# microsoft/GenerativeImage2Text

Hardware: AMD Instinct MI355X
Metric: captions/sec whole-node (GIT_BASE 224px bs=64/GPU greedy len=20) (higher is better)
Workload: dtype f16; 1 GPU; GIT_BASE 224px bs=64/GPU greedy max_len=20 frames=1; global_batch=64, parallelism=dp1, decode_steps_per_caption=19, seq_len_returned=20, hip_graph=True, contexts_in_flight=4, layernorm_folded=True, library=libgitmi_f16.so, encoder_chains=2, schedule=mixed

## Files before the change

### generativeimage2text_amd/csrc/kernels_attn.hip

```cpp
#include "gitmi_common.h"
#include "launchers.h"
#include <type_traits>

namespace gitmi {

constexpr int HD = 64;

template <typename T>
__global__ __launch_bounds__(256) void attn_full_valu_kernel(AttnFullArgs a) {
    __shared__ float Ks[64][HD + 1];
    __shared__ float Vs[64][HD + 1];
    __shared__ float qs[16][HD];
    __shared__ float ps[16][64];

    const int tid = threadIdx.x, lane = tid & 63, wave = tid >> 6;
    const int h = blockIdx.y, b = blockIdx.z;
    const int q0 = blockIdx.x * 16;
    const T* Q = reinterpret_cast<const T*>(a.q);
    const T* K = reinterpret_cast<const T*>(a.k);
    const T* V = reinterpret_cast<const T*>(a.v);
    T* O = reinterpret_cast<T*>(a.out);
    const size_t base_row = (size_t)b * a.N;
    const int n = a.ntok ? a.ntok[b] : a.N;
    if (q0 >= n) {
// ... 49 lines not shown
            for (int key = 0; key < 64; ++key) o += ps[qi][key] * Vs[key][lane];
            o_acc[j] = o;
        }
    }
#pragma unroll
    for (int j = 0; j < 4; ++j) {
        const int qr = q0 + wave * 4 + j;
        if (qr < a.N) st<T>(O + (base_row + qr) * a.ldo + h * HD + lane, qr < n ? o_acc[j] / l_run[j] : 0.f);
    }
}

constexpr int FA_LDK = HD + 8;
constexpr int FA_LDV = 64 + 8;

__global__ __launch_bounds__(256) void attn_full_mfma_kernel(AttnFullArgs a) {
    __shared__ __attribute__((aligned(16))) bf16_t Ks[64 * FA_LDK];
    __shared__ __attribute__((aligned(16))) bf16_t Vt[HD * FA_LDV];

    constexpr int QT = 4;
    const int tid = threadIdx.x, lane = tid & 63, wave = tid >> 6;
    const int l15 = lane & 15, lg = lane >> 4;
    const int h = blockIdx.y, b = blockIdx.z;
    const int qbase = blockIdx.x * 256;
    const bf16_t* Q = reinterpret_cast<const bf16_t*>(a.q);
    const bf16_t* K = reinterpret_cast<const bf16_t*>(a.k);
    const bf16_t* V = reinterpret_cast<const bf16_t*>(a.v);
    bf16_t* O = reinterpret_cast<bf16_t*>(a.out);
    const size_t base_row = (size_t)b * a.N;
    const int n = a.ntok ? a.ntok[b] : a.N;

    bf16x8_t qf[QT][2];
    f32x4_t o_acc[QT][4];
    float m_run[QT], l_run[QT];
#pragma unroll
    for (int t = 0; t < QT; ++t) {
        int qr = qbase + (t * 4 + wave) * 16 + l15;
        qr = qr < n ? qr : n - 1;
        const bf16_t* qp = Q + (base_row + qr) * a.ldq + h * HD + lg * 8;
        qf[t][0] = *reinterpret_cast<const bf16x8_t*>(qp);
        qf[t][1] = *reinterpret_cast<const bf16x8_t*>(qp + 32);
#pragma unroll
        for (int dt = 0; dt < 4; ++dt) o_acc[t][dt] = f32x4_t{0.f, 0.f, 0.f, 0.f};
        m_run[t] = -INFINITY;
        l_run[t] = 0.f;
    }

    const int ld_row = tid >> 3;
    const int ld_c = (tid & 7) * 8;

    const int kend = qbase < n ? n : 0;
    for (int kt = 0; kt < kend; kt += 64) {
        __syncthreads();
#pragma unroll
        for (int it = 0; it < 2; ++it) {
            const int key = ld_row + it * 32;
            int kr = kt + key;
            kr = kr < n ? kr : n - 1;
            const u32x4_t kc = *reinterpret_cast<const u32x4_t*>(K + (base_row + kr) * a.ldk + h * HD + ld_c);
            const u32x4_t vc = *reinterpret_cast<const u32x4_t*>(V + (base_row + kr) * a.ldv + h * HD + ld_c);
            *reinterpret_cast<u32x4_t*>(Ks + key * FA_LDK + ld_c) = kc;
#pragma unroll
            for (int e = 0; e < 4; ++e) {
                Vt[(ld_c + 2 * e) * FA_LDV + key] = (bf16_t)(vc[e] & 0xffffu);
                Vt[(ld_c + 2 * e + 1) * FA_LDV + key] = (bf16_t)(vc[e] >> 16);
            }
        }
        __syncthreads();

#pragma unroll
        for (int t = 0; t < QT; ++t) {
            if (qbase + (t * 4 + wave) * 16 >= n) continue;
            f32x4_t s_acc[4];
#pragma unroll
            for (int st_ = 0; st_ < 4; ++st_) {
                s_acc[st_] = f32x4_t{0.f, 0.f, 0.f, 0.f};
#pragma unroll
                for (int ks = 0; ks < 2; ++ks) {
                    const bf16x8_t kf = *reinterpret_cast<const bf16x8_t*>(Ks + (st_ * 16 + l15) * FA_LDK + ks * 32 + lg * 8);
                    s_acc[st_] = mfma16(kf, qf[t][ks], s_acc[st_]);
                }
            }
            float tmax = -INFINITY;
#pragma unroll
            for (int st_ = 0; st_ < 4; ++st_)
#pragma unroll
                for (int r = 0; r < 4; ++r) {
                    const int key = kt + st_ * 16 + lg * 4 + r;
                    const float sv = key < n ? s_acc[st_][r] * a.scale : -INFINITY;
                    s_acc[st_][r] = sv;
                    tmax = fmaxf(tmax, sv);
                }
            tmax = fmaxf(tmax, __shfl_xor(tmax, 16, 64));
            tmax = fmaxf(tmax, __shfl_xor(tmax, 32, 64));
            const float m_new = fmaxf(m_run[t], tmax);
            const float alpha = fast_exp(m_run[t] - m_new);
            float psum = 0.f;
#pragma unroll
            for (int st_ = 0; st_ < 4; ++st_)
#pragma unroll
                for (int r = 0; r < 4; ++r) {
                    const float p = fast_exp(s_acc[st_][r] - m_new);
                    s_acc[st_][r] = p;
                    psum += p;
                }
            psum += __shfl_xor(psum, 16, 64);
            psum += __shfl_xor(psum, 32, 64);
            l_run[t] = l_run[t] * alpha + psum;
            m_run[t] = m_new;
#pragma unroll
            for (int dt = 0; dt < 4; ++dt)
#pragma unroll
                for (int r = 0; r < 4; ++r) o_acc[t][dt][r] *= alpha;

#pragma unroll
            for (int hf = 0; hf < 2; ++hf) {
                bf16x8_t pf;
                {
                    union { bf16x8_t v; uint32_t u[4]; } pk;
                    pk.u[0] = pack2bf(s_acc[2 * hf][0], s_acc[2 * hf][1]);
                    pk.u[1] = pack2bf(s_acc[2 * hf][2], s_acc[2 * hf][3]);
                    pk.u[2] = pack2bf(s_acc[2 * hf + 1][0], s_acc[2 * hf + 1][1]);
                    pk.u[3] = pack2bf(s_acc[2 * hf + 1][2], s_acc[2 * hf + 1][3]);
                    pf = pk.v;
                }
#pragma unroll
                for (int dt = 0; dt < 4; ++dt) {
                    union { bf16x8_t v; uint2 h2[2]; } vf;
                    const bf16_t* vp = Vt + (dt * 16 + l15) * FA_LDV + hf * 32 + lg * 4;
                    vf.h2[0] = *reinterpret_cast<const uint2*>(vp);
                    vf.h2[1] = *reinterpret_cast<const uint2*>(vp + 16);
                    o_acc[t][dt] = mfma16(vf.v, pf, o_acc[t][dt]);
                }
            }
        }
    }

#pragma unroll
    for (int t = 0; t < QT; ++t) {
        const int qr = qbase + (t * 4 + wave) * 16 + l15;
        if (qr < a.N) {
            const float inv = qr < n ? 1.0f / l_run[t] : 0.f;
            bf16_t* op = O + (base_row + qr) * a.ldo + h * HD;
#pragma unroll
            for (int dt = 0; dt < 4; ++dt) {
                uint2 tt;
                tt.x = pack2bf(o_acc[t][dt][0] * inv, o_acc[t][dt][1] * inv);
                tt.y = pack2bf(o_acc[t][dt][2] * inv, o_acc[t][dt][3] * inv);
                *reinterpret_cast<uint2*>(op + dt * 16 + lg * 4) = tt;
            }
        }
    }
}

template <int NSUB, bool RAGGED = false>
__global__ __launch_bounds__(256, 2) void attn_full_mfma_short_kernel(AttnFullArgs a) {
    constexpr int NK = NSUB * 16;
    constexpr int NB = (NSUB + 1) / 2;
    constexpr int LDV = NB * 32 + 8;
    static_assert((LDV / 8) % 2 == 1, "V^T row stride must be an odd multiple of 16 bytes");
    __shared__ __attribute__((aligned(16))) bf16_t Ks[NK * FA_LDK];
    __shared__ __attribute__((aligned(16))) bf16_t Vt[HD * LDV];

    const int tid = threadIdx.x, lane = tid & 63, wave = tid >> 6;
    const int l15 = lane & 15, lg = lane >> 4;
    const int h = blockIdx.x, b = blockIdx.y;
    const bf16_t* Q = reinterpret_cast<const bf16_t*>(a.q);
    const bf16_t* K = reinterpret_cast<const bf16_t*>(a.k);
    const bf16_t* V = reinterpret_cast<const bf16_t*>(a.v);
    bf16_t* O = reinterpret_cast<bf16_t*>(a.out);
    const size_t base_row = (size_t)b * a.N;
    const int n = RAGGED ? a.ntok[b] : a.N;
    if constexpr (RAGGED) {
        for (int i = tid; i < (a.N - n) * 8; i += 256) {
            const int qr = n + (i >> 3);
            *reinterpret_cast<u32x4_t*>(O + (base_row + qr) * a.ldo + h * HD + (i & 7) * 8) = u32x4_t{0u, 0u, 0u, 0u};
        }
    }

#pragma unroll
    for (int it = 0; it < (NK * 8 + 255) / 256; ++it) {
        int idx = tid + it * 256;
        const bool ok = idx < NK * 8;
        idx = ok ? idx : NK * 8 - 1;
        const int key = idx >> 3, c = idx & 7;
        const int kr = key < n ? key : n - 1;
        const u32x4_t kc = *reinterpret_cast<const u32x4_t*>(K + (base_row + kr) * a.ldk + h * HD + c * 8);
        if (ok) *reinterpret_cast<u32x4_t*>(Ks + key * FA_LDK + c * 8) = kc;
    }
#pragma unroll
    for (int it = 0; it < (NB * 8 * 8 + 255) / 256; ++it) {
        int task = tid + it * 256;
        const bool ok = task < NB * 8 * 8;
        task = ok ? task : NB * 8 * 8 - 1;
        const int kg = task % (NB * 8), c = task / (NB * 8);
        u32x4_t vc[4];
#pragma unroll
        for (int e = 0; e < 4; ++e) {
            const int key = kg * 4 + e;
            const int kr = key < n ? key : n - 1;
            vc[e] = *reinterpret_cast<const u32x4_t*>(V + (base_row + kr) * a.ldv + h * HD + c * 8);
            if (key >= n) vc[e] = u32x4_t{0u, 0u, 0u, 0u};
        }
        if (ok) {
#pragma unroll
            for (int w = 0; w < 4; ++w) {
                uint2 even, odd;
                even.x = (vc[0][w] & 0xffffu) | (vc[1][w] << 16);
                even.y = (vc[2][w] & 0xffffu) | (vc[3][w] << 16);
                odd.x = (vc[0][w] >> 16) | (vc[1][w] & 0xffff0000u);
                odd.y = (vc[2][w] >> 16) | (vc[3][w] & 0xffff0000u);
                *reinterpret_cast<uint2*>(Vt + (c * 8 + 2 * w) * LDV + kg * 4) = even;
                *reinterpret_cast<uint2*>(Vt + (c * 8 + 2 * w + 1) * LDV + kg * 4) = odd;
            }
        }
    }
    __syncthreads();

    const int nqt = (n + 15) >> 4;
    const float c2 = a.scale * 1.4426950408889634f;

    auto process = [&](auto nt_c, int t0) {
        constexpr int NT = decltype(nt_c)::value;
        bf16x8_t qf[NT][2];
#pragma unroll
        for (int u = 0; u < NT; ++u) {
            int qr = (t0 + 4 * u) * 16 + l15;
            qr = qr < n ? qr : n - 1;
            const bf16_t* qp = Q + (base_row + qr) * a.ldq + h * HD + lg * 8;
            qf[u][0] = *reinterpret_cast<const bf16x8_t*>(qp);
            qf[u][1] = *reinterpret_cast<const bf16x8_t*>(qp + 32);
        }
        f32x4_t sacc[NT][NSUB];
#pragma unroll
        for (int st_ = 0; st_ < NSUB; ++st_) {
            const bf16x8_t kf0 = *reinterpret_cast<const bf16x8_t*>(Ks + (st_ * 16 + l15) * FA_LDK + lg * 8);
            const bf16x8_t kf1 = *reinterpret_cast<const bf16x8_t*>(Ks + (st_ * 16 + l15) * FA_LDK + 32 + lg * 8);
#pragma unroll
            for (int u = 0; u < NT; ++u) {
                sacc[u][st_] = mfma16(kf0, qf[u][0], f32x4_t{0.f, 0.f, 0.f, 0.f});
                sacc[u][st_] = mfma16(kf1, qf[u][1], sacc[u][st_]);
            }
            if constexpr (NSUB > 13) { if (st_ % 4 == 3) __builtin_amdgcn_sched_barrier(0); }
        }
        float inv_l[NT];
#pragma unroll
        for (int u = 0; u < NT; ++u) {
            if constexpr (RAGGED) {
#pragma unroll
                for (int st_ = 0; st_ < NSUB; ++st_)
#pragma unroll
                    for (int r = 0; r < 4; ++r)
                        if (st_ * 16 + lg * 4 + r >= n) sacc[u][st_][r] = -INFINITY;
            } else {
#pragma unroll
                for (int r = 0; r < 4; ++r)
                    if ((NSUB - 1) * 16 + lg * 4 + r >= a.N) sacc[u][NSUB - 1][r] = -INFINITY;
            }
            float m = -INFINITY;
#pragma unroll
            for (int st_ = 0; st_ < NSUB; ++st_)
#pragma unroll
                for (int r = 0; r < 4; ++r) m = fmaxf(m, sacc[u][st_][r]);
            m = fmaxf(m, __shfl_xor(m, 16, 64));
            m = fmaxf(m, __shfl_xor(m, 32, 64));
            const float mc = m * c2;
            float psum = 0.f;
#pragma unroll
            for (int st_ = 0; st_ < NSUB; ++st_)
#pragma unroll
                for (int r = 0; r < 4; ++r) {
                    const float p = __builtin_amdgcn_exp2f(sacc[u][st_][r] * c2 - mc);
                    sacc[u][st_][r] = p;
                    psum += p;
                }
            psum += __shfl_xor(psum, 16, 64);
            psum += __shfl_xor(psum, 32, 64);
            inv_l[u] = 1.0f / psum;
        }
        uint32_t pk2[NT][NSUB][2];
#pragma unroll
        for (int u = 0; u < NT; ++u)
#pragma unroll
            for (int st_ = 0; st_ < NSUB; ++st_) {
                pk2[u][st_][0] = pack2bf(sacc[u][st_][0], sacc[u][st_][1]);
                pk2[u][st_][1] = pack2bf(sacc[u][st_][2], sacc[u][st_][3]);
            }
        f32x4_t o_acc[NT][4];
#pragma unroll
        for (int u = 0; u < NT; ++u)
#pragma unroll
            for (int dt = 0; dt < 4; ++dt) o_acc[u][dt] = f32x4_t{0.f, 0.f, 0.f, 0.f};
#pragma unroll
        for (int blk = 0; blk < NB; ++blk) {
            bf16x8_t pf[NT];
#pragma unroll
            for (int u = 0; u < NT; ++u) {
                union { bf16x8_t v; uint32_t w[4]; } pk;
                pk.w[0] = pk2[u][2 * blk][0];
                pk.w[1] = pk2[u][2 * blk][1];
                const bool has1 = 2 * blk + 1 < NSUB;
                const int s1 = has1 ? 2 * blk + 1 : 0;
                pk.w[2] = has1 ? pk2[u][s1][0] : 0u;
                pk.w[3] = has1 ? pk2[u][s1][1] : 0u;
                pf[u] = pk.v;
            }
#pragma unroll
            for (int dt = 0; dt < 4; ++dt) {
                union { bf16x8_t v; uint2 h2[2]; } vf;
                const bf16_t* vp = Vt + (dt * 16 + l15) * LDV + blk * 32 + lg * 4;
                vf.h2[0] = *reinterpret_cast<const uint2*>(vp);
                vf.h2[1] = *reinterpret_cast<const uint2*>(vp + 16);
#pragma unroll
                for (int u = 0; u < NT; ++u)
                    o_acc[u][dt] = mfma16(vf.v, pf[u], o_acc[u][dt]);
            }
        }
#pragma unroll
        for (int u = 0; u < NT; ++u) {
            const int qr = (t0 + 4 * u) * 16 + l15;
            if (qr < n) {
                bf16_t* op = O + (base_row + qr) * a.ldo + h * HD;
#pragma unroll
                for (int dt = 0; dt < 4; ++dt) {
                    uint2 tt;
                    tt.x = pack2bf(o_acc[u][dt][0] * inv_l[u], o_acc[u][dt][1] * inv_l[u]);
                    tt.y = pack2bf(o_acc[u][dt][2] * inv_l[u], o_acc[u][dt][3] * inv_l[u]);
                    *reinterpret_cast<uint2*>(op + dt * 16 + lg * 4) = tt;
                }
            }
        }
    };

    for (int t0 = wave; t0 < nqt; t0 += 8) {
        if (t0 + 4 < nqt) process(std::integral_constant<int, 2>{}, t0);
        else process(std::integral_constant<int, 1>{}, t0);
    }
}

template <typename T>
__global__ void kv_repack_kernel(const T* __restrict__ qkv, T* __restrict__ kh, T* __restrict__ vh, int B, int N, int H,
                                 int d) {
    constexpr int CH = 16 / (int)sizeof(T);
    constexpr int CPH = HD / CH;
    const size_t per = (size_t)B * H * N * CPH;
    for (size_t i = blockIdx.x * (size_t)blockDim.x + threadIdx.x; i < 2 * per; i += (size_t)gridDim.x * blockDim.x) {
        const int kv = i >= per;
        size_t r = kv ? i - per : i;
        const int c = (int)(r % CPH); r /= CPH;
        const int n = (int)(r % N); r /= N;
        const int h = (int)(r % H);
        const int b = (int)(r / H);
        const T* src = qkv + ((size_t)b * N + n) * 3 * d + (kv ? 2 : 1) * d + h * HD + c * CH;
        T* dst = (kv ? vh : kh) + (((size_t)b * H + h) * N + n) * HD + c * CH;
        *reinterpret_cast<u32x4_t*>(dst) = *reinterpret_cast<const u32x4_t*>(src);
    }
}

template <typename T> struct Raw8;
template <> struct Raw8<bf16_t> {
    u32x4_t r;
    __device__ __forceinline__ void load(const bf16_t* p) { r = *reinterpret_cast<const u32x4_t*>(p); }
    __device__ __forceinline__ void load_nt(const bf16_t* p) { r = __builtin_nontemporal_load(reinterpret_cast<const u32x4_t*>(p)); }
    __device__ __forceinline__ void store(bf16_t* p) const { *reinterpret_cast<u32x4_t*>(p) = r; }
    __device__ __forceinline__ void zero() { r = u32x4_t{0u, 0u, 0u, 0u}; }
    __device__ __forceinline__ void get(float (&v)[8]) const {
#pragma unroll
        for (int i = 0; i < 4; ++i) {
            unpack2op(r[i], v[2 * i], v[2 * i + 1]);
        }
    }
};
template <> struct Raw8<float> {
    f32x4_t a, b;
    __device__ __forceinline__ void load(const float* p) {
        a = *reinterpret_cast<const f32x4_t*>(p);
        b = *reinterpret_cast<const f32x4_t*>(p + 4);
    }
    __device__ __forceinline__ void load_nt(const float* p) {
        a = __builtin_nontemporal_load(reinterpret_cast<const f32x4_t*>(p));
        b = __builtin_nontemporal_load(reinterpret_cast<const f32x4_t*>(p + 4));
    }
    __device__ __forceinline__ void store(float* p) const {
        *reinterpret_cast<f32x4_t*>(p) = a;
        *reinterpret_cast<f32x4_t*>(p + 4) = b;
    }
    __device__ __forceinline__ void zero() { a = f32x4_t{0.f, 0.f, 0.f, 0.f}; b = a; }
    __device__ __forceinline__ void get(float (&v)[8]) const {
#pragma unroll
        for (int i = 0; i < 4; ++i) { v[i] = a[i]; v[4 + i] = b[i]; }
    }
};

template <typename T, int KB, int PF = 8, int TI = 5>
__global__ __launch_bounds__(256) void attn_decode_kernel(AttnDecodeArgs a) {
    __shared__ float part[4][KB][HD + 2];

    const int tid = threadIdx.x;
    const int h = blockIdx.x, b = blockIdx.y, H = gridDim.x;
    const int k = a.beams;
    const T* QKV = reinterpret_cast<const T*>(a.qkv);
    const T* IMGK = reinterpret_cast<const T*>(a.img_k);
    const T* IMGV = reinterpret_cast<const T*>(a.img_v);
    T* TK = reinterpret_cast<T*>(a.txt_k);
    T* TV = reinterpret_cast<T*>(a.txt_v);
    T* O = reinterpret_cast<T*>(a.out);
    const int ld3 = 3 * a.d;
    const int row0 = b * k;
    const int grp = tid >> 3, sub = tid & 7;
    const int wave = tid >> 6;

    const int bi = a.img_of ? a.img_of[b] : b;
    const int n_img = a.ntok ? a.ntok[bi] : a.N_img;
    const T* kbase = IMGK + ((size_t)bi * H + h) * a.N_img * HD + sub * 8;
    const T* vbase = IMGV + ((size_t)bi * H + h) * a.N_img * HD + sub * 8;
    const int nt = a.pos + 1;

    int t_j[TI], t_s[TI], t_row[TI];
#pragma unroll
    for (int u = 0; u < TI; ++u) {
        const int it = grp + 32 * u;
        t_j[u] = it < k * nt ? it / nt : -1;
        t_s[u] = it < k * nt ? it % nt : 0;
        if constexpr (KB == 1) t_row[u] = row0;
        else t_row[u] = (t_j[u] >= 0 && t_s[u] != a.pos) ? a.kv_src[(size_t)(row0 + t_j[u]) * a.ld_src + t_s[u]] : 0;
    }
    Raw8<T> qr[KB];
#pragma unroll
    for (int j = 0; j < KB; ++j) {
        if (j < k) qr[j].load(QKV + (size_t)(row0 + j) * ld3 + h * HD + sub * 8);
        else qr[j].zero();
    }
    Raw8<T> kr[PF], vr[PF];
#pragma unroll
    for (int u = 0; u < PF; ++u) {
        const int n = grp + 32 * u;
        if (n < n_img && !(a.dbg & 1)) { kr[u].load_nt(kbase + (size_t)n * HD); vr[u].load_nt(vbase + (size_t)n * HD); }
        else { kr[u].zero(); vr[u].zero(); }
    }
    Raw8<T> tk[TI], tv[TI];
#pragma unroll
    for (int u = 0; u < TI; ++u) {
        if (t_j[u] < 0) { tk[u].zero(); tv[u].zero(); }
        else if (t_s[u] == a.pos) {
            const T* src = QKV + (size_t)(row0 + t_j[u]) * ld3 + a.d + h * HD + sub * 8;
            tk[u].load(src);
            tv[u].load(src + a.d);
        } else {
            const size_t off = ((size_t)t_row[u] * a.T_max + t_s[u]) * a.d + h * HD + sub * 8;
            tk[u].load(TK + off);
            tv[u].load(TV + off);
        }
    }
    if (tid < k * 8) {
        const int j = tid >> 3;
        const T* src = QKV + (size_t)(row0 + j) * ld3 + a.d + h * HD + sub * 8;
        const size_t dst = ((size_t)(row0 + j) * a.T_max + a.pos) * a.d + h * HD + sub * 8;
        Raw8<T> ck, cv;
        ck.load(src);
        cv.load(src + a.d);
        ck.store(TK + dst);
        cv.store(TV + dst);
    }

    float q[KB][8], m[KB], l[KB], o[KB][8];
// ... 191 lines not shown
```

### generativeimage2text_amd/engine.py

```python
from __future__ import annotations

import ctypes as C
import os
from typing import Dict, List, Mapping, Optional, Sequence, Tuple

import torch

_HERE = os.path.dirname(os.path.abspath(__file__))
LIB_PATH = os.path.join(_HERE, "libgitmi.so")
LIB_PATH_F16 = os.path.join(_HERE, "libgitmi_f16.so")
LIB_PATH_EXP = os.path.join(_HERE, "libgitmi_exp.so")
LIB_PATH_F16_EXP = os.path.join(_HERE, "libgitmi_f16_exp.so")

PREC_BF16, PREC_F32 = 0, 1
DTYPE_F32, DTYPE_BF16, DTYPE_F16 = 0, 1, 2
DTYPE_F16_STREAM = 3
SEARCH_AUTOREGRESSIVE, SEARCH_GENERATOR, SEARCH_TRIE = 0, 1, 2
SEARCH_SCORE = 3
SEARCH_ATTEND = 4
SEARCH_CONTEXT = 5
SEARCH_TREE_SCORE = 6
ACT_NONE, ACT_QUICKGELU, ACT_GELU_ERF = 0, 1, 2

EXPORTED_SYMBOLS = [
# ... 909 lines not shown
def from_frag(xf: torch.Tensor, rows: int) -> torch.Tensor:
    Rp, K = xf.shape
    return xf.reshape(Rp // 16, K // 32, 4, 16, 8).permute(0, 3, 1, 2, 4).reshape(Rp, K)[:rows].contiguous()


def _pad_vec(v: Optional[torch.Tensor], n: int) -> Optional[torch.Tensor]:
    if v is None:
        return None
    out = torch.zeros(n, dtype=v.dtype, device=v.device)
    out[:v.numel()] = v
    return out


def op_dgemm(A: torch.Tensor, W: torch.Tensor, bias: torch.Tensor, colsum: Optional[torch.Tensor] = None,
             stats: Optional[torch.Tensor] = None, eps: float = 1e-12, act: int = ACT_NONE,
             frag_out: bool = False, packed: bool = False, strips_per_wg: int = 0) -> torch.Tensor:
    lib = _op_library(A.dtype, W.dtype)
    if packed:
        Af, Wf, M, N, K = A, W, int(A.shape[0]), int(bias.numel()), int(A.shape[1])
        if stats is not None:
            M = int(stats.shape[1])
    else:
        M, K = A.shape
        N = W.shape[0]
        Af, Wf = to_frag(A, 64), to_frag(W)
    out = torch.empty((M + 15) // 16 * 16 if frag_out else M, N, device=A.device, dtype=A.dtype)
    strips = 0 if stats is None else int(stats.shape[0])
    _ck(lib.gitmi_op_dgemm(Af.data_ptr(), Wf.data_ptr(), bias.data_ptr(), _ptr(colsum), _ptr(stats), strips, eps,
                           out.data_ptr(), 1 if frag_out else 0, M, N, K, act, int(strips_per_wg), _stream()), lib)
    return from_frag(out, M) if (frag_out and not packed) else out


def op_dgemm_res(A: torch.Tensor, W: torch.Tensor, bias: torch.Tensor, res_x: torch.Tensor,
                 res_stats: Optional[torch.Tensor] = None, res_gamma: Optional[torch.Tensor] = None,
                 res_beta: Optional[torch.Tensor] = None, res_eps: float = 1e-12, packed: bool = False):
    lib = _op_library(A.dtype, W.dtype)
    M, N = res_x.shape
    K = A.shape[1]
    Af, Wf = (A, W) if packed else (to_frag(A, 64), to_frag(W))
    x = torch.empty(M, N, device=A.device, dtype=torch.float32)
    xb = torch.empty((M + 15) // 16 * 16, (N + 31) // 32 * 32, device=A.device, dtype=A.dtype)
    st = torch.empty(N // 16, M, 2, device=A.device, dtype=torch.float32)
    strips = 0 if res_stats is None else int(res_stats.shape[0])
    _ck(lib.gitmi_op_dgemm_res(Af.data_ptr(), Wf.data_ptr(), bias.data_ptr(), res_x.data_ptr(), _ptr(res_stats), strips,
                               _ptr(res_gamma), _ptr(res_beta), res_eps, x.data_ptr(), xb.data_ptr(), st.data_ptr(),
                               M, N, K, _stream()), lib)
    return x, (xb if packed else from_frag(xb, M)[:, :N].contiguous()), st


def op_dgemm_form(A: torch.Tensor, W: torch.Tensor, bias: torch.Tensor, M: Optional[int] = None, *, colsum=None, stats=None,
                  eps: float = 1e-12, act: int = ACT_NONE, frag_out: bool = False, out: Optional[torch.Tensor] = None,
                  res_x=None, res_stats=None, res_gamma=None, res_beta=None, res_eps: float = 1e-12, x=None, xb=None,
                  stats_out=None, packed: bool = False, rows_per_wg: int = 0, strips_per_wg: int = 0, no_row_walk: int = 0):
    lib = _exp_library(A.dtype, W.dtype)
    own = A.dtype
    if own == torch.float32:
        raise GitmiError(f"operands must be bf16 or fp16, got {A.dtype} / {W.dtype}")
    if packed:
        if M is None:
            raise ValueError("packed operands: M is required")
        Af, Wf = A, W
    else:
        M = int(A.shape[0]) if M is None else int(M)
        Af, Wf = to_frag(A, 64), to_frag(W)
    M, N, K = int(M), int(bias.numel()), int(A.shape[1])
    Mp = (M + 15) // 16 * 16
    producer = res_x is not None
    if producer:
        x = torch.empty(M, N, device=A.device, dtype=torch.float32) if x is None else x
        xb = torch.empty(Mp, (N + 31) // 32 * 32, device=A.device, dtype=own) if xb is None else xb
        stats_out = torch.empty(N // 16, M, 2, device=A.device, dtype=torch.float32) if stats_out is None else stats_out
    elif out is None:
        out = torch.empty(Mp if frag_out else M, N, device=A.device, dtype=own)
    _ck(_experiment_only(lib, "gitmi_debug_dgemm_form")(
        Af.data_ptr(), int(Af.shape[0]), Wf.data_ptr(), _ptr(bias), _ptr(colsum), _ptr(stats),
        0 if stats is None else int(stats.shape[0]), eps, _ptr(out), int(bool(frag_out)), int(act), _ptr(res_x), _ptr(res_stats),
        0 if res_stats is None else int(res_stats.shape[0]), _ptr(res_gamma), _ptr(res_beta), res_eps, _ptr(x), _ptr(xb),
        _ptr(stats_out), M, N, K, int(rows_per_wg), int(strips_per_wg), int(no_row_walk), _stream()), lib)
    return (x, xb, stats_out) if producer else out


def _vocab_head_call(A, W, bias, mtop, cols_per_wg, colsum, stats, want_logits, packed, rows, V, measurement=False):
    lib = _exp_library(A.dtype, W.dtype) if measurement else _op_library(A.dtype, W.dtype)
    K = A.shape[1]
    V = int(bias.numel()) if V is None else int(V)
    if packed:
        Af, Wf, M, bp, cp = A, W, int(rows), bias, colsum
    else:
        M = A.shape[0]
        Vp = (V + cols_per_wg - 1) // cols_per_wg * cols_per_wg
        Af, Wf, bp, cp = to_frag(A, 64), to_frag(W, cols_per_wg), _pad_vec(bias, Vp), _pad_vec(colsum, Vp)
    nparts = (V + cols_per_wg - 1) // cols_per_wg
    slots = 1 if mtop <= 1 else 2 if mtop <= 2 else 4 if mtop <= 4 else 8 if mtop <= 8 else 16
    pv = torch.empty(M, nparts, slots, device=A.device, dtype=torch.float32)
    pi = torch.empty(M, nparts, slots, device=A.device, dtype=torch.int32)
    pl = torch.empty(M, nparts, 2, device=A.device, dtype=torch.float32)
    lg = torch.empty(M, V, device=A.device, dtype=torch.float32) if want_logits else None
    strips = 0 if stats is None else int(stats.shape[0])
    keep = (Af, Wf, bp, cp)
    return lib, M, (Af.data_ptr(), Wf.data_ptr(), bp.data_ptr(), _ptr(cp), _ptr(stats), strips), (M, V, K, cols_per_wg, mtop), \
        (pv.data_ptr(), pi.data_ptr(), pl.data_ptr(), _ptr(lg)), (pv, pi, pl, lg), keep


def op_vocab_topm(A: torch.Tensor, W: torch.Tensor, bias: torch.Tensor, mtop: int, cols_per_wg: int = 128,
                  colsum: Optional[torch.Tensor] = None, stats: Optional[torch.Tensor] = None, eps: float = 1e-12,
                  suppress_tok: Optional[torch.Tensor] = None, want_logits: bool = False, packed: bool = False,
                  rows: Optional[int] = None, V: Optional[int] = None, max_wgs: int = 0):
    lib, _, ops, shape, outs, result, keep = _vocab_head_call(A, W, bias, mtop, cols_per_wg, colsum, stats, want_logits, packed, rows, V)
    _ck(lib.gitmi_op_vocab_topm(*ops, eps, *shape, _ptr(suppress_tok), *outs, int(max_wgs), _stream()), lib)
    return result


def op_vocab_topm_rules(A: torch.Tensor, W: torch.Tensor, bias: torch.Tensor, mtop: int, ids: Optional[torch.Tensor],
                        cur_len: int, plen: Optional[torch.Tensor], beams: int = 1, suppress_kind: int = 0,
                        rep_penalty: float = 0.0, cols_per_wg: int = 128, colsum: Optional[torch.Tensor] = None,
                        stats: Optional[torch.Tensor] = None, eps: float = 1e-12, want_logits: bool = False, packed: bool = False,
                        rows: Optional[int] = None, V: Optional[int] = None, max_wgs: int = 0):
    lib, M, ops, shape, outs, result, keep = _vocab_head_call(A, W, bias, mtop, cols_per_wg, colsum, stats, want_logits, packed, rows, V,
                                                              measurement=True)
    if ids is not None:
        ids = ids.to(device=A.device, dtype=torch.int32).contiguous()
        plen = plen.to(device=A.device, dtype=torch.int32).contiguous()
        if ids.dim() != 2 or ids.shape[0] != M or plen.numel() * beams != M:
            raise ValueError(f"ids {tuple(ids.shape)} / plen {tuple(plen.shape)} do not describe {M} rows of {beams} beams")
    _ck(_experiment_only(lib, "gitmi_debug_vocab_topm_rules")(
        *ops, eps, *shape, _ptr(ids), 0 if ids is None else int(ids.shape[1]), int(cur_len), _ptr(plen), int(beams),
        int(suppress_kind), float(rep_penalty), *outs, int(max_wgs), _stream()), lib)
    return result


def set_gemm_impl(impl: int) -> None:
    global _gemm_impl
    lib = load_library()
    _ck(_experiment_only(lib, "gitmi_debug_set_gemm_impl")(int(impl)), lib)
    _gemm_impl = int(impl)
    other = _libs.get("f16_exp")
    if other is not None and other is not lib:
        _ck(other.gitmi_debug_set_gemm_impl(int(impl)), other)


def op_attn_decode(qkv, img_k, img_v, txt_k, txt_v, kv_src, B, H, N_img, T_max, pos, beams, dbg=0):
    lib = _op_library(qkv.dtype, img_k.dtype, img_v.dtype, txt_k.dtype, txt_v.dtype, fp32_ok=True)
    R, d = B * beams, H * 64
    out = torch.empty(R, d, device=qkv.device, dtype=qkv.dtype)
    if qkv.dtype != torch.float32 and img_k.dim() == 4:
        img_k, img_v = kv_repack(img_k, img_v)
    _ck(lib.gitmi_op_attn_decode(qkv.data_ptr(), img_k.data_ptr(), img_v.data_ptr(), txt_k.data_ptr(), txt_v.data_ptr(),
                                 kv_src.data_ptr(), out.data_ptr(), B, H, N_img, T_max, pos, beams, _torch_dtype_code(qkv),
                                 dbg, _stream()), lib)
    return out


def op_attention_ragged(qkv: torch.Tensor, ntok, B: int, N: int, H: int, impl: int) -> torch.Tensor:
    lib = load_library()
    nt = torch.as_tensor(ntok, dtype=torch.int32).to(qkv.device)
    out = torch.empty(B * N, H * 64, device=qkv.device, dtype=qkv.dtype)
    _ck(_experiment_only(lib, "gitmi_debug_attention_ragged")(qkv.data_ptr(), out.data_ptr(), nt.data_ptr(), B, N, H,
                                                              _torch_dtype_code(qkv), impl, _stream()), lib)
    return out


def op_attn_decode_ragged(qkv, img_k, img_v, txt_k, txt_v, kv_src, ntok, B, H, N_img, T_max, pos, beams):
    lib = load_library()
    R, d = B * beams, H * 64
    nt = torch.as_tensor(ntok, dtype=torch.int32).to(qkv.device)
    out = torch.empty(R, d, device=qkv.device, dtype=qkv.dtype)
    if qkv.dtype != torch.float32 and img_k.dim() == 4:
        img_k, img_v = kv_repack(img_k, img_v)
    _ck(_experiment_only(lib, "gitmi_debug_attn_decode_ragged")(qkv.data_ptr(), img_k.data_ptr(), img_v.data_ptr(), txt_k.data_ptr(),
                                                                txt_v.data_ptr(), kv_src.data_ptr(), out.data_ptr(), nt.data_ptr(), B,
                                                                H, N_img, T_max, pos, beams, _torch_dtype_code(qkv), _stream()), lib)
    return out


def op_attn_decode_form(qkv, img_k, img_v, txt_k, txt_v, kv_src, B, H, N_img, T_max, pos, beams, *, out=None, img_of=None,
                        ntok=None, out_frag=False, pairs_per_wg=0, waves_per_pair=0, stream_wgs=0, operands=None):
    lib = _exp_library(qkv.dtype, img_k.dtype, img_v.dtype, txt_k.dtype, txt_v.dtype,
                       operands=operands if qkv.dtype == torch.float32 else None)
    R, d = B * beams, H * 64
    n_images = img_k.shape[0] if img_k.dim() == 4 else img_k.numel() // (H * ((N_img + 31) // 32 * 32) * 64)
    if qkv.dtype != torch.float32 and img_k.dim() == 4:
        img_k, img_v = kv_repack(img_k, img_v)
    if img_of is None:
        if n_images < B:
            raise ValueError(f"{n_images} images for {B} sentences and no img_of")
    else:
        host = torch.as_tensor(img_of, dtype=torch.int64).cpu()
        if host.numel() != B or int(host.min()) < 0 or int(host.max()) >= n_images:
            raise ValueError(f"img_of {host.tolist()} does not map {B} sentences onto {n_images} images")
        img_of = host.to(device=qkv.device, dtype=torch.int32)
    if ntok is not None:
        ntok = torch.as_tensor(ntok, dtype=torch.int32).to(qkv.device)
        if ntok.numel() != n_images:
            raise ValueError(f"ntok holds {ntok.numel()} counts for {n_images} images")
    if out is None:
        rows = (R + 15) // 16 * 16 if out_frag else R
        out = torch.empty(rows, d, device=qkv.device, dtype=qkv.dtype)
    _ck(_experiment_only(lib, "gitmi_debug_attn_decode_form")(
        qkv.data_ptr(), img_k.data_ptr(), img_v.data_ptr(), txt_k.data_ptr(), txt_v.data_ptr(), kv_src.data_ptr(), out.data_ptr(),
        _ptr(ntok), _ptr(img_of), n_images, B, H, N_img, T_max, pos, beams, _torch_dtype_code(qkv), int(bool(out_frag)),
        int(pairs_per_wg), int(waves_per_pair), int(stream_wgs), _stream()), lib)
    return out


def op_attn_decode_qkv(x, w, bias, img_k, img_v, txt_k, txt_v, kv_src, B, H, N_img, T_max, pos, beams=1, *, colsum=None, stats=None,
                       eps: float = 1e-12, out=None, img_of=None, ntok=None, out_frag=False, pairs_per_wg=8, waves_per_pair=1,
                       stream_wgs=0):
    lib = _exp_library(x.dtype, w.dtype, img_k.dtype, img_v.dtype, txt_k.dtype, txt_v.dtype)
    d = H * 64
    n_images = img_k.shape[0] if img_k.dim() == 4 else img_k.numel() // (H * ((N_img + 31) // 32 * 32) * 64)
    if img_k.dim() == 4:
        img_k, img_v = kv_repack(img_k, img_v)
    if img_of is not None:
        img_of = torch.as_tensor(img_of, dtype=torch.int32).to(x.device)
    if ntok is not None:
        ntok = torch.as_tensor(ntok, dtype=torch.int32).to(x.device)
    if out is None:
        out = torch.empty((B * beams + 15) // 16 * 16 if out_frag else B * beams, d, device=x.device, dtype=x.dtype)
    _ck(_experiment_only(lib, "gitmi_debug_attn_decode_qkv")(
        x.data_ptr(), int(x.shape[0]), w.data_ptr(), _ptr(bias), _ptr(colsum), _ptr(stats), 0 if stats is None else int(stats.shape[0]),
        eps, img_k.data_ptr(), img_v.data_ptr(), txt_k.data_ptr(), txt_v.data_ptr(), kv_src.data_ptr(), out.data_ptr(), _ptr(ntok),
        _ptr(img_of), n_images, B, H, N_img, T_max, pos, beams, _torch_dtype_code(x), int(bool(out_frag)), int(pairs_per_wg),
        int(waves_per_pair), int(stream_wgs), _stream()), lib)
    return out


def op_score_attn(qkv: torch.Tensor, img_kv: torch.Tensor, image_of: torch.Tensor, Q: int, H: int, N_img: int,
                  Lp: int) -> torch.Tensor:
    lib = load_library()
    img = image_of.to(device=qkv.device, dtype=torch.int32).contiguous()
    out = torch.empty(Q * Lp, H * 64, device=qkv.device, dtype=qkv.dtype)
    _ck(_experiment_only(lib, "gitmi_debug_score_attn")(qkv.data_ptr(), img_kv.data_ptr(), img.data_ptr(), out.data_ptr(), Q, H,
                                                        N_img, Lp, _torch_dtype_code(qkv), _stream()), lib)
    return out


def op_score_attn_map(qkv: torch.Tensor, img_kv: torch.Tensor, image_of: torch.Tensor, Q: int, H: int, N_img: int, Lp: int,
                      ntok: Optional[torch.Tensor] = None) -> torch.Tensor:
    lib = load_library()
    img = image_of.to(device=qkv.device, dtype=torch.int32).contiguous()
    nt = None if ntok is None else ntok.to(device=qkv.device, dtype=torch.int32).contiguous()
    out = torch.empty(Q, Lp, N_img + Lp, device=qkv.device, dtype=torch.float32)
    _ck(_experiment_only(lib, "gitmi_debug_score_attn_map")(qkv.data_ptr(), img_kv.data_ptr(), img.data_ptr(), _ptr(nt),
                                                            out.data_ptr(), Q, H, N_img, Lp, _torch_dtype_code(qkv), _stream()), lib)
    return out


def pack_trees(tokens, depths, lengths, vocab: int, max_depth: int):
    tok = torch.as_tensor(tokens).detach().to("cpu", torch.int64)
    dep = torch.as_tensor(depths).detach().to("cpu", torch.int64)
    if tok.dim() != 2 or tok.shape[1] < 1 or dep.shape != tok.shape:
        raise ValueError(f"tokens and depths must both be [Q, L], got {tuple(tok.shape)} and {tuple(dep.shape)}")
    Q, L = int(tok.shape[0]), int(tok.shape[1])
    lens = [L] * Q if lengths is None else [int(v) for v in lengths]
    if len(lens) != Q:
        raise ValueError(f"lengths has {len(lens)} entries for {Q} trees")
    for q, n in enumerate(lens):
        if n < 1 or n > L:
            raise ValueError(f"tree {q}: length {n} outside [1, {L}]")
    valid = torch.arange(L)[None, :] < torch.as_tensor(lens)[:, None]
    first = dep[:, 0] != 0
    if bool(first.any()):
        q = int(first.nonzero()[0])
        raise ValueError(f"tree {q}, node 0: the root must have depth 0, got {int(dep[q, 0])}")
    step = torch.zeros_like(valid)
    step[:, 1:] = (dep[:, 1:] < 1) | (dep[:, 1:] > dep[:, :-1] + 1)
    for wrong, what in ((step & valid, "must lie in [1, depth of the node before it + 1] (one root; a child is one level below)"),
                        ((dep >= max_depth) & valid, f"must be below {max_depth} (min(max_text_len, max_pos))")):
        if bool(wrong.any()):
            q, i = (int(v) for v in wrong.nonzero()[0])
            raise ValueError(f"tree {q}, node {i}: depth {int(dep[q, i])} {what}")
    ids = tok[valid]
    if int(ids.min()) < 0 or int(ids.max()) >= vocab:
        raise ValueError(f"token ids outside [0, {vocab})")
    table = torch.where(valid, (dep << 32) | tok, torch.zeros_like(tok)).contiguous()
    return table, lens


def op_score_attn_tree(qkv: torch.Tensor, img_kv: torch.Tensor, image_of: torch.Tensor, table: torch.Tensor, lens, max_depth: int,
                       Q: int, H: int, N_img: int, Lp: int, ntok: Optional[torch.Tensor] = None):
    lib = load_library()
    dev = qkv.device
    img = image_of.to(device=dev, dtype=torch.int32).contiguous()
    nt = None if ntok is None else ntok.to(device=dev, dtype=torch.int32).contiguous()
    tab = table.to(device=dev, dtype=torch.int64).contiguous()
    ln = torch.as_tensor(lens).to(device=dev, dtype=torch.int32).contiguous()
    if tuple(tab.shape) != (Q, Lp) or ln.numel() != Q:
        raise ValueError("table must be [Q, Lp] and lens [Q]")
    out = torch.empty(Q * Lp, H * 64, device=dev, dtype=qkv.dtype)
    bad = torch.empty(Q, device=dev, dtype=torch.int32)
    _ck(_experiment_only(lib, "gitmi_debug_score_attn_tree")(qkv.data_ptr(), img_kv.data_ptr(), img.data_ptr(), _ptr(nt),
                                                             tab.data_ptr(), ln.data_ptr(), max_depth, out.data_ptr(),
                                                             bad.data_ptr(), Q, H, N_img, Lp, _torch_dtype_code(qkv), _stream()),
        lib)
    return out, bad


def op_score_head(A: torch.Tensor, W: torch.Tensor, bias: torch.Tensor, tgt: torch.Tensor) -> torch.Tensor:
    lib = load_library()
    M, K = A.shape
    V = W.shape[0]
    t = tgt.to(device=A.device, dtype=torch.int32).contiguous()
    out = torch.zeros(M, 2, device=A.device, dtype=torch.float32)
    _ck(_experiment_only(lib, "gitmi_debug_score_head")(A.data_ptr(), W.data_ptr(), bias.float().contiguous().data_ptr(),
                                                        t.data_ptr(), M, V, K, _torch_dtype_code(A), out.data_ptr(),
                                                        _stream()), lib)
    return out
# ... 115 lines not shown
```

Baseline: 11380 captions/s.

## Swizzle K/V shared layouts, prefetch Q, raise occupancy in short attention kernel

Replaces the padded K and transposed-V shared-memory layouts with XOR-swizzled compact layouts, which shrinks LDS use and avoids bank conflicts. It issues all K and V global loads before the LDS stores and prefetches the next Q tile into registers during the PV phase. It also raises the occupancy hint to three workgroups per CU for short non-ragged sequences. The costs are more register pressure from the held K/V/Q values and more complex index math. The ragged debug path now loads from the experimental library.

```diff
diff --git a/generativeimage2text_amd/csrc/kernels_attn.hip b/generativeimage2text_amd/csrc/kernels_attn.hip
--- a/generativeimage2text_amd/csrc/kernels_attn.hip
+++ b/generativeimage2text_amd/csrc/kernels_attn.hip
@@ -225,14 +225,18 @@
     }
 }
 
+__device__ __forceinline__ int fa_k_off(int key, int c) { return key * HD + ((c ^ (key & 7)) << 3); }
+__device__ __forceinline__ int fa_vt_off(int st, int dt, int lg, int l15) {
+    return ((((st * 4 + dt) * 4 + lg) << 4) + (l15 ^ ((lg & 1) | (dt << 1)))) << 2;
+}
+
 template <int NSUB, bool RAGGED = false>
-__global__ __launch_bounds__(256, 2) void attn_full_mfma_short_kernel(AttnFullArgs a) {
+__global__ __launch_bounds__(256, (NSUB <= 13 && !RAGGED) ? 3 : 2) void attn_full_mfma_short_kernel(AttnFullArgs a) {
     constexpr int NK = NSUB * 16;
     constexpr int NB = (NSUB + 1) / 2;
-    constexpr int LDV = NB * 32 + 8;
-    static_assert((LDV / 8) % 2 == 1, "V^T row stride must be an odd multiple of 16 bytes");
-    __shared__ __attribute__((aligned(16))) bf16_t Ks[NK * FA_LDK];
-    __shared__ __attribute__((aligned(16))) bf16_t Vt[HD * LDV];
+    __shared__ __attribute__((aligned(16))) bf16_t Ks[NK * HD];
+    __shared__ __attribute__((aligned(16))) bf16_t Vt[HD * NK];
+    static_assert(NSUB > 13 || sizeof(Ks) + sizeof(Vt) <= 53248, "three workgroups per CU need at most 53 248 B each");
 
     const int tid = threadIdx.x, lane = tid & 63, wave = tid >> 6;
     const int l15 = lane & 15, lg = lane >> 4;
@@ -250,64 +254,91 @@
         }
     }
 
-#pragma unroll
-    for (int it = 0; it < (NK * 8 + 255) / 256; ++it) {
+    const int nqt = (n + 15) >> 4;
+    bf16x8_t qn[2][2];
+    const bf16_t* Qh = Q + base_row * a.ldq + h * HD;
+    auto request_q = [&](int t0) {
+#pragma unroll
+        for (int u = 0; u < 2; ++u) {
+            if (u == 0 || t0 + 4 < nqt) {
+                int qr = (t0 + 4 * u) * 16 + l15;
+                qr = qr < n ? qr : n - 1;
+                const bf16_t* qp = Qh + (unsigned)(qr * a.ldq + lg * 8);
+                qn[u][0] = *reinterpret_cast<const bf16x8_t*>(qp);
+                qn[u][1] = *reinterpret_cast<const bf16x8_t*>(qp + 32);
+            }
+        }
+    };
+    qn[1][0] = qn[1][1] = bf16x8_t{};
+    if (wave < nqt) request_q(wave);
+
+    constexpr int KIT = (NK * 8 + 255) / 256, VIT = (NSUB * 4 * 8 + 255) / 256;
+    static_assert(NK * 8 >= 256 && NSUB * 4 * 8 >= 256, "the wrapped lanes need a full first pass");
+    u32x4_t kc[KIT], vc[VIT][4];
+#pragma unroll
+    for (int it = 0; it < KIT; ++it) {
         int idx = tid + it * 256;
-        const bool ok = idx < NK * 8;
-        idx = ok ? idx : NK * 8 - 1;
+        idx = idx < NK * 8 ? idx : idx - NK * 8;
         const int key = idx >> 3, c = idx & 7;
         const int kr = key < n ? key : n - 1;
-        const u32x4_t kc = *reinterpret_cast<const u32x4_t*>(K + (base_row + kr) * a.ldk + h * HD + c * 8);
-        if (ok) *reinterpret_cast<u32x4_t*>(Ks + key * FA_LDK + c * 8) = kc;
-    }
-#pragma unroll
-    for (int it = 0; it < (NB * 8 * 8 + 255) / 256; ++it) {
+        kc[it] = *reinterpret_cast<const u32x4_t*>(K + (base_row + kr) * a.ldk + h * HD + c * 8);
+    }
+#pragma unroll
+    for (int it = 0; it < VIT; ++it) {
         int task = tid + it * 256;
-        const bool ok = task < NB * 8 * 8;
-        task = ok ? task : NB * 8 * 8 - 1;
-        const int kg = task % (NB * 8), c = task / (NB * 8);
-        u32x4_t vc[4];
+        task = task < NSUB * 4 * 8 ? task : task - NSUB * 4 * 8;
+        const int c = task & 7, kg = task >> 3;
 #pragma unroll
         for (int e = 0; e < 4; ++e) {
             const int key = kg * 4 + e;
             const int kr = key < n ? key : n - 1;
-            vc[e] = *reinterpret_cast<const u32x4_t*>(V + (base_row + kr) * a.ldv + h * HD + c * 8);
-            if (key >= n) vc[e] = u32x4_t{0u, 0u, 0u, 0u};
-        }
-        if (ok) {
-#pragma unroll
-            for (int w = 0; w < 4; ++w) {
-                uint2 even, odd;
-                even.x = (vc[0][w] & 0xffffu) | (vc[1][w] << 16);
-                even.y = (vc[2][w] & 0xffffu) | (vc[3][w] << 16);
-                odd.x = (vc[0][w] >> 16) | (vc[1][w] & 0xffff0000u);
-                odd.y = (vc[2][w] >> 16) | (vc[3][w] & 0xffff0000u);
-                *reinterpret_cast<uint2*>(Vt + (c * 8 + 2 * w) * LDV + kg * 4) = even;
-                *reinterpret_cast<uint2*>(Vt + (c * 8 + 2 * w + 1) * LDV + kg * 4) = odd;
-            }
+            vc[it][e] = *reinterpret_cast<const u32x4_t*>(V + (base_row + kr) * a.ldv + h * HD + c * 8);
+        }
+    }
+#pragma unroll
+    for (int it = 0; it < KIT; ++it) {
+        int idx = tid + it * 256;
+        idx = idx < NK * 8 ? idx : idx - NK * 8;
+        *reinterpret_cast<u32x4_t*>(Ks + fa_k_off(idx >> 3, idx & 7)) = kc[it];
+    }
+#pragma unroll
+    for (int it = 0; it < VIT; ++it) {
+        int task = tid + it * 256;
+        task = task < NSUB * 4 * 8 ? task : task - NSUB * 4 * 8;
+        const int c = task & 7, kg = task >> 3;
+#pragma unroll
+        for (int e = 0; e < 4; ++e)
+            if (kg * 4 + e >= n) vc[it][e] = u32x4_t{0u, 0u, 0u, 0u};
+#pragma unroll
+        for (int w = 0; w < 4; ++w) {
+            uint2 even, odd;
+            even.x = (vc[it][0][w] & 0xffffu) | (vc[it][1][w] << 16);
+            even.y = (vc[it][2][w] & 0xffffu) | (vc[it][3][w] << 16);
+            odd.x = (vc[it][0][w] >> 16) | (vc[it][1][w] & 0xffff0000u);
+            odd.y = (vc[it][2][w] >> 16) | (vc[it][3][w] & 0xffff0000u);
+            *reinterpret_cast<uint2*>(Vt + fa_vt_off(kg >> 2, c >> 1, kg & 3, (c & 1) * 8 + 2 * w)) = even;
+            *reinterpret_cast<uint2*>(Vt + fa_vt_off(kg >> 2, c >> 1, kg & 3, (c & 1) * 8 + 2 * w + 1)) = odd;
         }
     }
     __syncthreads();
 
-    const int nqt = (n + 15) >> 4;
     const float c2 = a.scale * 1.4426950408889634f;
+    const bf16_t* krd[2] = {Ks + fa_k_off(l15, lg), Ks + fa_k_off(l15, 4 + lg)};
+    const int vrd0 = fa_vt_off(0, 0, lg, l15);
 
     auto process = [&](auto nt_c, int t0) {
         constexpr int NT = decltype(nt_c)::value;
         bf16x8_t qf[NT][2];
 #pragma unroll
         for (int u = 0; u < NT; ++u) {
-            int qr = (t0 + 4 * u) * 16 + l15;
-            qr = qr < n ? qr : n - 1;
-            const bf16_t* qp = Q + (base_row + qr) * a.ldq + h * HD + lg * 8;
-            qf[u][0] = *reinterpret_cast<const bf16x8_t*>(qp);
-            qf[u][1] = *reinterpret_cast<const bf16x8_t*>(qp + 32);
+            qf[u][0] = qn[u][0];
+            qf[u][1] = qn[u][1];
         }
         f32x4_t sacc[NT][NSUB];
 #pragma unroll
         for (int st_ = 0; st_ < NSUB; ++st_) {
-            const bf16x8_t kf0 = *reinterpret_cast<const bf16x8_t*>(Ks + (st_ * 16 + l15) * FA_LDK + lg * 8);
-            const bf16x8_t kf1 = *reinterpret_cast<const bf16x8_t*>(Ks + (st_ * 16 + l15) * FA_LDK + 32 + lg * 8);
+            const bf16x8_t kf0 = *reinterpret_cast<const bf16x8_t*>(krd[0] + st_ * 16 * HD);
+            const bf16x8_t kf1 = *reinterpret_cast<const bf16x8_t*>(krd[1] + st_ * 16 * HD);
 #pragma unroll
             for (int u = 0; u < NT; ++u) {
                 sacc[u][st_] = mfma16(kf0, qf[u][0], f32x4_t{0.f, 0.f, 0.f, 0.f});
@@ -363,15 +394,23 @@
         for (int u = 0; u < NT; ++u)
 #pragma unroll
             for (int dt = 0; dt < 4; ++dt) o_acc[u][dt] = f32x4_t{0.f, 0.f, 0.f, 0.f};
+        __builtin_amdgcn_sched_barrier(0);
+        if (t0 + 8 < nqt) request_q(t0 + 8);
+        __builtin_amdgcn_sched_barrier(0);
+        int vb = vrd0;
+        asm volatile("" : "+v"(vb));
+        const bf16_t* vrd[4];
+#pragma unroll
+        for (int dt = 0; dt < 4; ++dt) vrd[dt] = Vt + dt * 4 * HD + (vb ^ (dt << 3));
 #pragma unroll
         for (int blk = 0; blk < NB; ++blk) {
+            const bool has1 = 2 * blk + 1 < NSUB;
             bf16x8_t pf[NT];
 #pragma unroll
             for (int u = 0; u < NT; ++u) {
                 union { bf16x8_t v; uint32_t w[4]; } pk;
                 pk.w[0] = pk2[u][2 * blk][0];
                 pk.w[1] = pk2[u][2 * blk][1];
-                const bool has1 = 2 * blk + 1 < NSUB;
                 const int s1 = has1 ? 2 * blk + 1 : 0;
                 pk.w[2] = has1 ? pk2[u][s1][0] : 0u;
                 pk.w[3] = has1 ? pk2[u][s1][1] : 0u;
@@ -380,9 +419,8 @@
 #pragma unroll
             for (int dt = 0; dt < 4; ++dt) {
                 union { bf16x8_t v; uint2 h2[2]; } vf;
-                const bf16_t* vp = Vt + (dt * 16 + l15) * LDV + blk * 32 + lg * 4;
-                vf.h2[0] = *reinterpret_cast<const uint2*>(vp);
-                vf.h2[1] = *reinterpret_cast<const uint2*>(vp + 16);
+                vf.h2[0] = *reinterpret_cast<const uint2*>(vrd[dt] + 2 * blk * 16 * HD);
+                vf.h2[1] = has1 ? *reinterpret_cast<const uint2*>(vrd[dt] + (2 * blk + 1) * 16 * HD) : uint2{0u, 0u};
 #pragma unroll
                 for (int u = 0; u < NT; ++u)
                     o_acc[u][dt] = mfma16(vf.v, pf[u], o_acc[u][dt]);
diff --git a/generativeimage2text_amd/engine.py b/generativeimage2text_amd/engine.py
--- a/generativeimage2text_amd/engine.py
+++ b/generativeimage2text_amd/engine.py
@@ -1085,7 +1085,7 @@
 
 
 def op_attention_ragged(qkv: torch.Tensor, ntok, B: int, N: int, H: int, impl: int) -> torch.Tensor:
-    lib = load_library()
+    lib = _exp_library(qkv.dtype)
     nt = torch.as_tensor(ntok, dtype=torch.int32).to(qkv.device)
     out = torch.empty(B * N, H * 64, device=qkv.device, dtype=qkv.dtype)
     _ck(_experiment_only(lib, "gitmi_debug_attention_ragged")(qkv.data_ptr(), out.data_ptr(), nt.data_ptr(), B, N, H,
```

Result: faster. 11520 captions/s (median of 6 runs) (+1.2%).
